# szumanski/Audio-Modem-Radio

Hardware: AMD Instinct MI355X
Metric: demod Msymbols/s (batch) + achieved HBM GB/s, QPSK@9600/96kHz, 1/2/4/8 GPU (higher is better)
Workload: dtype f64; 1 GPU; qpsk9600; global_batch=4096, batches_in_flight=16, steps_per_launch=1, streams_per_launch=4096, kernel_layout=lane, hw_queues=32

## Files before the change

audio-modem-radio_amd/build.py:

```python
from __future__ import annotations

import hashlib
import os
import subprocess
import sys

HERE = os.path.dirname(os.path.abspath(__file__))
CSRC = os.path.join(HERE, "csrc")
INCLUDE = os.path.join(os.path.dirname(HERE), "include")
LIB = os.path.join(HERE, "libamr.so")
LIB_ID = LIB + ".id"
SOURCES = ["psk_kernels.hip", "psk_lane_kernels.hip", "psk_split_kernels.hip", "psk_soft_kernels.hip", "psk8_kernels.hip", "util_kernels.hip", "fft_kernels.hip", "fsk_kernels.hip", "fsk_exact_kernels.hip", "pocketfft_kernels.hip", "frame_kernels.hip", "tx_kernels.hip",
           "hell_kernels.hip", "viterbi_kernels.hip", "rs_kernels.hip", "ofdm_kernels.hip", "ofdm_acq_kernels.hip", "dsss_kernels.hip", "dsss_acq_kernels.hip", "msk_kernels.hip", "msk_acq_kernels.hip", "tone8_kernels.hip", "tone8_acq_kernels.hip", "api.cpp", "tx_api.cpp", "hell_api.cpp",
           "viterbi_api.cpp", "rs_api.cpp", "ofdm_api.cpp", "dsss_api.cpp", "msk_api.cpp", "tone8_api.cpp", "fsk_api.cpp", "pocketfft_plan.cpp"]
HEADERS = ["amr_internal.h", "psk_common.h", "fft.h", "api_common.h", "plan_core.h", "sym_plan.h", "tx_host.h", "env_switch.h", "dev_mem.h", "fsk_exact.h", "pocketfft.h", "pocketfft_dev.h",
           "iir_design.h", "split_chain.h", "split_bound.h", "odd_ext.h", "split_strict.h", "hell.h", "hell_glyphs.h", "viterbi.h", "rs.h", "ofdm.h", "dsss.h", "msk.h", "tone8.h", os.path.join(INCLUDE, "amr.h")]
ARCH = os.environ.get("AMR_OFFLOAD_ARCH", "gfx950")
HIPCC = os.environ.get("HIPCC", "/opt/rocm/bin/hipcc")
CFLAGS = ["-O3", "-std=c++17", "-fPIC", "-ffp-contract=off", "-fno-fast-math", f"--offload-arch={ARCH}",
          "-I", CSRC, "-I", INCLUDE, "-Wall", "-Wno-unused-function"]


def _digest(paths, extra: str = "") -> str:
    h = hashlib.sha256()
    for p in paths:
        with open(p, "rb") as f:
            h.update(os.path.basename(p).encode() + b"\0" + f.read())
    h.update(extra.encode())
    return h.hexdigest()[:16]

# ... 65 lines not shown
```

audio-modem-radio_amd/csrc/api.cpp:

```cpp
#include <hip/hip_runtime.h>
#include <rccl/rccl.h>

#include <algorithm>
#include <cmath>
#include <cstdio>
#include <cstdlib>
#include <cstring>
#include <mutex>
#include <optional>
#include <string>
#include <tuple>
#include <vector>

#include "amr_internal.h"
#include "api_common.h"
#include "dev_mem.h"
#include "iir_design.h"
#include "plan_core.h"
#include "split_strict.h"

namespace amr {
hipError_t launch_psk_bandpass(const PskBuffers&, const PskParams&, const Iir&, hipStream_t);
hipError_t launch_psk_lowpass_fwd(const PskBuffers&, const PskParams&, const Iir&, hipStream_t);
hipError_t launch_psk_lowpass_bwd(const PskBuffers&, const PskParams&, const Iir&, hipStream_t);
hipError_t launch_psk_lowpass_exact(const PskBuffers&, const PskParams&, const Iir&, hipStream_t);
hipError_t launch_psk_slice(const PskBuffers&, const PskParams&, hipStream_t, bool only_flagged = false);
hipError_t launch_psk_soft(const PskBuffers&, const PskParams&, int8_t*, int64_t, hipStream_t);
hipError_t launch_psk_slice8(const PskBuffers&, const PskParams&, hipStream_t, bool only_flagged = false);
hipError_t launch_psk_soft8(const PskBuffers&, const PskParams&, int8_t*, int64_t, hipStream_t);
hipError_t launch_psk_bandpass_lane(const PskBuffers&, const PskParams&, const Iir&, hipStream_t);
hipError_t launch_psk_bandpass_fixup(const PskBuffers&, const PskParams&, const Iir&, hipStream_t);
bool psk_lane_fused(const PskBuffers&, const PskParams&);
hipError_t launch_psk_lowpass_lane(const PskBuffers&, const PskParams&, const Iir&, hipStream_t, bool* sliced, int* kernel);
int64_t psk_lane_bp_scratch_doubles(int64_t n_streams, int64_t n, int pad);
int64_t psk_lane_lp_scratch_doubles(int64_t n_streams, int64_t n, int pad);
int64_t psk_exact_scratch_bytes(int64_t n_streams, int64_t m2);
hipError_t launch_synth_tile_noise(const float*, int64_t, int64_t, float*, int64_t, int64_t, float, uint64_t,
                                   hipStream_t);
hipError_t launch_sync_pack_gated(const uint32_t*, int64_t, int64_t, int64_t, uint8_t*, int64_t, int64_t*, int64_t*,
                                  const int32_t*, hipStream_t);
hipError_t launch_psk_split_bp(const PskBuffers&, const PskParams&, const Iir&, const PskSplit&, hipStream_t);
hipError_t launch_psk_split_lp(const PskBuffers&, const PskParams&, const Iir&, const PskSplit&, hipStream_t);
hipError_t launch_psk_split_slice(const PskBuffers&, const PskParams&, const PskSplit&, hipStream_t);
hipError_t launch_fec_decode(const uint8_t*, int64_t, const int64_t*, int64_t, uint8_t*, int64_t, int64_t*,
                             int32_t*, const uint32_t*, const uint32_t*, hipStream_t);
hipError_t launch_frame_parse(const uint8_t*, int64_t, const int64_t*, int64_t, int64_t, int32_t*, amr_frame_rec*,
                              const uint32_t*, const uint32_t*, hipStream_t);
}
// ... 943 lines not shown
    HIP_TRY(psk_slice_kind(b, pl->p, st));
    if (!gated) HIP_TRY(gate_wait(pl->gate, st));
    HIP_TRY(psk_sync_pack(pl, c.io, b.words, b.gate));
    if (c.soft.ptr) HIP_TRY(psk_soft_kind(b, pl->p, c.soft.ptr, c.soft.stride, st));
    return AMR_OK;
  });
}

int run_psk_lane(amr_psk_plan* pl, const PskCall& c, PskBuffers b) {
  hipStream_t st = pl->stream;
  static const bool f32f_env = env_on("AMR_PSK_F32F");
  static const bool nofix = env_on("AMR_PSK_F32F_NOFIX");
  b.fpeak = reinterpret_cast<double*>(pl->mem.split_peak.as<unsigned long long>());
  b.f32f = f32f_env && pl->p.f32_margin > 0.0 && !pl->lp_exact_only && psk_lane_fused(b, pl->p) ? 1 : 0;
  pl->last_f32f = b.f32f != 0;
  HIP_TRY_TIMED(*pl, AMR_T_BANDPASS, launch_psk_bandpass_lane(b, pl->p, pl->bp, st));
  bool sliced = false;
  if (pl->lp_exact_only) {
    HIP_TRY(hipMemsetD32Async((hipDeviceptr_t)b.flags, 1, (size_t)c.io.B, st));
  } else {
    HIP_TRY_TIMED(*pl, AMR_T_LOWPASS_FWD, launch_psk_lowpass_lane(b, pl->p, pl->lp, st, &sliced, &pl->last_lowpass));
  }
  if (int rc = timed(*pl, AMR_T_LOWPASS_EXACT, [&]() -> int {
        if (b.f32f && !nofix) HIP_TRY(launch_psk_bandpass_fixup(b, pl->p, pl->bp, st));
        HIP_TRY(launch_psk_lowpass_exact(b, pl->p, pl->lp, st));
        return AMR_OK;
      }))
    return rc;
  return timed(*pl, AMR_T_SYNC_PACK, [&]() -> int {
    HIP_TRY(psk_slice_kind(b, pl->p, st, sliced));
// ... 565 lines not shown
```

audio-modem-radio_amd/csrc/psk_kernels.hip:

```cpp
#include <math.h>
#include <stdlib.h>

#include <type_traits>

#include "amr_internal.h"
#include "psk_common.h"

namespace amr {

constexpr int kTileBytes = 256;
constexpr int kTilePitch = kTileBytes + 16;
constexpr int kBwdChunk = 32;

template <int CTRL>
__device__ __forceinline__ double dpp_f64(double v) {
  const long long u = __builtin_bit_cast(long long, v);
  const int lo = __builtin_amdgcn_mov_dpp((int)(u & 0xffffffff), CTRL, 0xF, 0xF, true);
  const int hi = __builtin_amdgcn_mov_dpp((int)(u >> 32), CTRL, 0xF, 0xF, true);
  return __builtin_bit_cast(double, ((long long)hi << 32) | (unsigned)lo);
}
constexpr int kQuadBcast0 = 0x00;

constexpr int kRowStreams = 4;
constexpr int kBpRing = 8;
// ... 729 lines not shown
        load(rr_[u]);
        __builtin_amdgcn_sched_barrier(0);
      }
    }
#pragma unroll
    for (int u = 0; u < R; ++u)
      if (cc - u >= 0) run(rr_[u], cc - u);
  }
  for (int jj = pad - 1; jj >= 0; --jj) {
    const double y = quad5_step(c, z, s3[s3q_index(w, comp, m2_pairs, jj + qs, sq)]);
    acc = tiny_min3(acc, y, y);
  }
  quad_flag(buf, s, j, !(acc >= kTinyHi) || !__builtin_isfinite(z));
}

template <int NT>
__device__ __forceinline__ void df2t_cplx_step(double (&zr)[NT - 1], double (&zc)[NT - 1],
                                               const double (&b)[NT], const double (&a)[NT],
                                               double x0, double x1, double& y0, double& y1) {
  const double t0x = 0.0 * x1, t1x = 0.0 * x0;
  y0 = zr[0] + (b[0] * x0 - t0x);
  y1 = zc[0] + (t1x + b[0] * x1);
  const double t0y = 0.0 * y1, t1y = 0.0 * y0;
#pragma unroll
  for (int i = 0; i < NT - 2; ++i) {
    const double r = zr[i + 1] + (b[i + 1] * x0 - t0x);
    const double m = zc[i + 1] + (t1x + b[i + 1] * x1);
    zr[i] = r - (a[i + 1] * y0 - t0y);
    zc[i] = m - (t1y + a[i + 1] * y1);
  }
  zr[NT - 2] = (b[NT - 1] * x0 - t0x) - (a[NT - 1] * y0 - t0y);
  zc[NT - 2] = (t1x + b[NT - 1] * x1) - (t1y + a[NT - 1] * y1);
}

__device__ __forceinline__ void cmul_np(double ar, double ai, double br, double bi, double& re, double& im) {
  re = __builtin_fma(ar, br, -(ai * bi));
  im = __builtin_fma(ar, bi, ai * br);
}

constexpr int kExactSlots = 128;
constexpr int kExactTile = 32;
int64_t psk_exact_slots(int64_t n_streams) {
  const int64_t g = (n_streams + kWave - 1) / kWave;
  return g < kExactSlots ? g : kExactSlots;
}
int64_t psk_exact_scratch_bytes(int64_t n_streams, int64_t m2) {
  const int64_t tiles = (m2 + kExactTile - 1) / kExactTile;
  return psk_exact_slots(n_streams) * tiles * 8 * kWave * 8;
}

template <int NT>
__global__ __launch_bounds__(64) void k_lowpass_exact(PskBuffers buf, PskParams p, Iir f) {
  if (buf.gate && *buf.gate == 0) return;
  static_assert(NT == 5, "checkpoint layout holds 2 x 4 states");
  const int lane = threadIdx.x;
  const int64_t n_groups = (buf.n_streams + kWave - 1) / kWave;
  const int64_t n = p.n;
  const int64_t n2 = (n + 1) >> 1;
  const int pad = p.pad2;
  const int64_t m2 = p.m2;
  const int64_t S = p.n_sym;
  const int64_t tiles = (m2 + kExactTile - 1) / kExactTile;
  const double4* __restrict__ lo = reinterpret_cast<const double4*>(buf.lo);
  double* __restrict__ ck = buf.s3 + (size_t)blockIdx.x * tiles * 8 * kWave + lane;
  double* __restrict__ sym = buf.s1;
  __shared__ double2 tile_out[kExactTile][kWave];
  for (int64_t g = blockIdx.x; g < n_groups; g += gridDim.x) {
    const int64_t s = g * kWave + lane;
    const bool live = s < buf.n_streams && buf.flags[s] != 0;
    if (!__any(live)) continue;

    double b[NT], a[NT], zr[NT - 1], zc[NT - 1];
#pragma unroll
    for (int i = 0; i < NT; ++i) { b[i] = f.b[i]; a[i] = f.a[i]; }

    auto bb = [&](int64_t i) -> double2 {
      const double fv = buf.s2[f_index(g, n2, i, lane)];
      const double4 l = lo[i];
      return make_double2(__builtin_fma(fv, l.x, l.y), __builtin_fma(fv, l.z, l.w));
    };
    const double2 x0 = bb(0), xl = bb(n - 1);
    double l2r, l2i, r2r, r2i;
    cmul_np(2.0, 0.0, x0.x, x0.y, l2r, l2i);
    cmul_np(2.0, 0.0, xl.x, xl.y, r2r, r2i);
    auto ext = [&](int64_t j) -> double2 {
      if (j < pad) { const double2 v = bb(pad - j); return make_double2(l2r - v.x, l2i - v.y); }
      if (j < pad + n) return bb(j - pad);
      const double2 v = bb(n - 2 - (j - pad - n));
      return make_double2(r2r - v.x, r2i - v.y);
    };
    {
      const double2 e0 = ext(0);
#pragma unroll
      for (int i = 0; i < NT - 1; ++i) cmul_np(f.zi[i], 0.0, e0.x, e0.y, zr[i], zc[i]);
    }
    double y0 = 0, y1 = 0;
    for (int64_t t = 0; t < tiles; ++t) {
      double* c = ck + (size_t)t * 8 * kWave;
#pragma unroll
      for (int i = 0; i < NT - 1; ++i) { c[i * kWave] = zr[i]; c[(NT - 1 + i) * kWave] = zc[i]; }
      const int64_t j1 = (t + 1) * kExactTile < m2 ? (t + 1) * kExactTile : m2;
      for (int64_t j = t * kExactTile; j < j1; ++j) {
        const double2 e = ext(j);
        df2t_cplx_step<NT>(zr, zc, b, a, e.x, e.y, y0, y1);
      }
    }
    double wr[NT - 1], wc[NT - 1];
#pragma unroll
    for (int i = 0; i < NT - 1; ++i) cmul_np(f.zi[i], 0.0, y0, y1, wr[i], wc[i]);

    int64_t k = S - 1;
    int64_t next_n = p.first + k * p.sps;
    for (int64_t t = tiles - 1; t >= 0; --t) {
      const double* c = ck + (size_t)t * 8 * kWave;
#pragma unroll
      for (int i = 0; i < NT - 1; ++i) { zr[i] = c[i * kWave]; zc[i] = c[(NT - 1 + i) * kWave]; }
      const int64_t j0 = t * kExactTile;
      const int64_t j1 = j0 + kExactTile < m2 ? j0 + kExactTile : m2;
      for (int64_t j = j0; j < j1; ++j) {
        const double2 e = ext(j);
        double o0, o1;
        df2t_cplx_step<NT>(zr, zc, b, a, e.x, e.y, o0, o1);
        tile_out[j - j0][lane] = make_double2(o0, o1);
      }
      for (int64_t j = j1 - 1; j >= j0; --j) {
        const double2 e = tile_out[j - j0][lane];
        double o0, o1;
        df2t_cplx_step<NT>(wr, wc, b, a, e.x, e.y, o0, o1);
        if (j - pad == next_n && k >= 0) {
          if (live) {
            sym[sym_index(s, S, k, 0)] = o0;
            sym[sym_index(s, S, k, 1)] = o1;
          }
          --k;
          next_n -= p.sps;
        }
      }
    }
  }
}

constexpr int kSliceWords = 32;
template <int WV>
__global__ __launch_bounds__(64 * WV) void k_slice(PskBuffers buf, PskParams p, int only_flagged) {
  if (buf.gate && *buf.gate == 0) return;
  constexpr int WPW = kSliceWords / WV;
  __shared__ uint32_t wl[kWave][kSliceWords + 1];
  const int lane = threadIdx.x & 63;
  const int wv = threadIdx.x >> 6;
  const int64_t s = (int64_t)blockIdx.y * kWave + lane;
  const bool live = s < buf.n_streams && (!only_flagged || buf.flags[s] != 0);
  const int64_t S = p.n_sym;
  const bool qpsk = p.kind == kQpsk;
// ... 120 lines not shown
```

audio-modem-radio_amd/csrc/psk_lane_kernels.hip:

```cpp
#include <math.h>

#include <type_traits>
#include <utility>

#include "amr.h"
#include "amr_internal.h"
#include "env_switch.h"
#include "psk_common.h"

namespace amr {

constexpr int kBpT = 32;
constexpr int kLpT = 40;
constexpr int kLpStaticFirstMax = 20;
constexpr int kLpCkReserveT = 20;


constexpr int kZoY = 1, kZoZ = 2;
template <int ZO>
__device__ __forceinline__ double bp_step(double (&z)[8], const Iir& f, double x, float& acc) {
  if constexpr (ZO == kZoZ) return df2t_step_zo(z, f, x, acc);
  else if constexpr (ZO == kZoY) return bp_step_zo(z, f, x);
  else return df2t_step<8>(z, f, x);
}
// ... 16 lines not shown
int64_t psk_lane_bp_scratch_doubles(int64_t n_streams, int64_t n, int pad) {
  const int64_t g = (n_streams + 63) / 64;
  return g * ((n / kBpT) * 8 + bp_lane_edge_cap(pad)) * 64;
}
int64_t psk_lane_lp_scratch_doubles(int64_t n_streams, int64_t n, int pad) {
  const int64_t g = (n_streams + 63) / 64;
  return 2 * g * ((n / kLpCkReserveT) * 4 + lp_lane_edge_cap(pad)) * 64;
}

template <typename T, int GPB, int ZO, bool FIXUP = false, bool F32F = false, int NT = 0>
__global__ __launch_bounds__(128 * GPB) void k_bp_lane2(PskBuffers buf, PskParams p, Iir f, int dev_fence) {
  static_assert(FIXUP ? GPB == 1 && !ZO && !F32F : GPB == 2,
                "two groups per workgroup, or the fix-up pass: one group, every tap, float64 f");
  static_assert(NT == 0 || !F32F, "cache policies: the float64 paths only");
  constexpr bool NTF = (NT & kNtFStore) != 0, NTC = (NT & kNtCk) != 0, NTX = (NT & kNtX) != 0;
  constexpr int TB = kBpT;
  constexpr int PER = 16 / (int)sizeof(T);
  constexpr int NL = TB / PER;
  static_assert(TB % PER == 0 && TB % 2 == 0, "tile = whole loads and whole pairs");
  __shared__ __attribute__((aligned(16))) double2 yb[GPB][2][TB / 2][64];
  const int lane = threadIdx.x & 63;
  const int wv = __builtin_amdgcn_readfirstlane(threadIdx.x >> 6);
  const int gi = wv >> 1, role = wv & 1;
  const int64_t w = (int64_t)blockIdx.x * GPB + gi;
  const bool active = w * 64 < buf.n_streams;
  const int64_t last = buf.n_streams - 1;
  const int64_t s = w * 64 + lane;
  if constexpr (FIXUP) {
    if (!active) return;
    if (!__syncthreads_or(s <= last && buf.bp_flags[s] != 0)) return;
// ... 52 lines not shown
        const double y1 = bp_step<ZO>(z, f, tile_x(cur, k + 1), acc);
        bp_watch<ZO>(acc, y0, y1);
      }
    }
    int e = 0;
    for (int64_t i = i_tail; i < n; ++i) {
      const double y = bp_step<ZO>(z, f, In<T>::cvt(x[i]), acc);
      bp_watch<ZO>(acc, y, y);
      st_pol<NTC>(&eb[(e++) * 64], y);
    }
    for (int jj = 0; jj < pad; ++jj) {
      const double y = bp_step<ZO>(z, f, ox.right(jj), acc);
      bp_watch<ZO>(acc, y, y);
      st_pol<NTC>(&eb[(e++) * 64], y);
    }
    if (bp_bad<ZO>(acc, z) && s <= last) atomicOr(&buf.bp_flags[s], 1);
    lane_pass_fence(dev_fence);
  }
  __syncthreads();

  if (role == 0) {
    v4u xr[NL];
    double cn[8];
    if (active && nt > 0) {
      load_tile(nt - 1, xr);
#pragma unroll
      for (int j = 0; j < 8; ++j) cn[j] = ld_pol<NTC>(&ck[((nt - 1) * 8 + j) * 64]);
    }
    for (int64_t it = 0; it <= nt; ++it) {
      const int64_t t = nt - 1 - it;
      if (active && t >= 0) {
// ... 16 lines not shown
          ybuf[k >> 1][lane] = make_double2(y0, y1);
        }
      }
      __syncthreads();
    }
  } else {
    double zb[8];
    float acc = __builtin_inff();
    unsigned long long pk = 0;
    auto pk_acc = [&](double y) {
      if constexpr (F32F) {
        const unsigned long long b = (unsigned long long)__double_as_longlong(y) & 0x7fffffffffffffffULL;
        pk = b > pk ? b : pk;
      }
    };
    if (active) {
      const double ylast = ld_pol<NTC>(&eb[(ne - 1) * 64]);
#pragma unroll
      for (int j = 0; j < 8; ++j) zb[j] = f.zi[j] * ylast;
      for (int e = ne - 1; e >= 0; --e) {
        const double y = bp_step<ZO>(zb, f, ld_pol<NTC>(&eb[e * 64]), acc);
        bp_watch<ZO>(acc, y, y);
        const int64_t i = i_tail + e;
        if (i < n) {
          if constexpr (F32F) {
            fo32[(i >> 1) * 64 + (i & 1)] = (float)y;
            pk_acc(y);
          } else {
            st_pol<NTF>(&fo[(i >> 1) * 64 + (i & 1)], y);
          }
        }
// ... 11 lines not shown
          const double2 yy = ybuf[k][lane];
          const double y1 = bp_step<ZO>(zb, f, yy.y, acc);
          const double y0 = bp_step<ZO>(zb, f, yy.x, acc);
          bp_watch<ZO>(acc, y1, y0);
          if constexpr (F32F) {
            *reinterpret_cast<float2*>(fp32 + k * 64) = make_float2((float)y0, (float)y1);
            pk_acc(y0);
            pk_acc(y1);
          } else {
            st_pair<NTF>(fp + k * 64, y0, y1);
          }
        }
      }
      __syncthreads();
    }
    if (active && bp_bad<ZO>(acc, zb) && s <= last) atomicOr(&buf.bp_flags[s], 1);
    if constexpr (F32F) {
      if (active && s <= last) buf.fpeak[s] = __longlong_as_double((long long)pk);
    }
  }
}

#ifndef AMR_LP_WAVES
#define AMR_LP_WAVES 1
#endif
#ifndef AMR_LP_CH
#define AMR_LP_CH 8
#endif
#ifndef AMR_LP_REGION_SYMS
#define AMR_LP_REGION_SYMS 8
#endif
template <int SPS, int FM, bool FUSE = false, bool F32F = false, int NT = 0>
__global__ __launch_bounds__(256, SPS > 0 ? AMR_LP_WAVES : 1) void k_lp_lane(PskBuffers buf, PskParams p, Iir f,
// ... 5 lines not shown
  static_assert(!F32F || FUSE, "the float32 hand-off's margin check runs in the fused slicer");
  using FV = typename std::conditional<F32F, float2, double2>::type;
  constexpr int TL = kLpT;
  constexpr int CH = AMR_LP_CH;
  constexpr int NCH = TL / CH, HC = CH / 2;
  constexpr int R = NCH % 2 == 0 ? NCH / 2 : NCH;
  static_assert(TL % CH == 0 && TL <= 64, "tile = whole chunks; one LO value per lane");
  static_assert(SPS == 0 || (TL % SPS == 0 && FM < SPS), "static symbol slots");
  __shared__ __attribute__((aligned(16))) double lo_lds[WPB][2][TL];
  constexpr int SPR = TL / (SPS > 0 ? SPS : TL);
  constexpr int MS = AMR_LP_REGION_SYMS;
  constexpr int RT = MS / SPR > 1 ? MS / SPR : 1;
  constexpr int NSL = FUSE ? 2 * MS : 1;
  static_assert(!FUSE || (RT * SPR <= MS && (MS & (MS - 1)) == 0), "a region holds at most MS symbols");
  __shared__ double sring[FUSE ? WPB : 1][NSL][64];
  const int lane = threadIdx.x & 63;
  const int wv = __builtin_amdgcn_readfirstlane(threadIdx.x >> 6);
  const int64_t w = (int64_t)blockIdx.x * (WPB / 2) + (wv >> 1);
  const int comp = wv & 1;
  const int64_t n = p.n, n2 = (n + 1) >> 1;
  const int pad = p.pad2;
  const int64_t nt = n / TL;
  if (w * 64 >= buf.n_streams) {
    if constexpr (FUSE) {
      for (int64_t b = 0; b < (nt > 1 ? (nt - 1 + RT - 1) / RT : 0) + 2; ++b) __syncthreads();
    }
    return;
  }
  const int64_t s = w * 64 + lane;
  const int64_t G = (buf.n_streams + 63) / 64;
// ... 223 lines not shown
        }
      }
      put_lo(tp, lop);
      if ((nt - 1 - t) % RT == RT - 1 || t == 1) {
        region_done(t * TL, r_hi);
        r_hi = t * TL;
      }
    }
  }
  for (int e = pad + (int)nh - 1; e >= 0; --e) {
    const double y = lp_step(zb, f, ld_pol<NTC>(&eh[e * 64]));
    accb = tiny_min3(accb, y, y);
    const int64_t i = e - pad;
    if (i >= 0) sym_out(i, y);
  }
  region_done(0, nh);
  bad |= !(accb >= kTinyHi);
#pragma unroll
  for (int j = 0; j < 4; ++j) bad |= !__builtin_isfinite(zb[j]);
  if constexpr (F32F) bad |= mflag;
  if (bad && s < buf.n_streams) {
    atomicOr(&buf.flags[s], 1);
    if constexpr (F32F) atomicOr(&buf.bp_flags[s], 1);
  }
}

template <int SPS, int FM, int NT = 0>
__global__ __launch_bounds__(256, AMR_LP_WAVES) void k_lp_lane_h(PskBuffers buf, PskParams p, Iir f, int dev_fence) {
  constexpr bool NTF = (NT & kNtFLoad) != 0, NTC = (NT & kNtCk) != 0, NTW = (NT & kNtWords) != 0;
  constexpr int TL = kLpT;
  constexpr int CH = AMR_LP_CH;
  constexpr int NCH = TL / CH, HC = CH / 2;
  constexpr int R = NCH % 2 == 0 ? NCH / 2 : NCH;
  static_assert(TL % CH == 0 && TL <= 64, "tile = whole chunks; one LO value of each component per lane");
  static_assert(SPS > 0 && TL % SPS == 0 && FM < SPS, "static symbol slots");
  __shared__ __attribute__((aligned(16))) double lo_lds[4][2][2][TL];
  const int lane = threadIdx.x & 63;
  const int hl = lane & 31, comp = lane >> 5;
// ... 205 lines not shown
        if (k % SPS == FM) slice(kt + (k - FM) / SPS, y1);
        if ((k - 1) % SPS == FM) slice(kt + (k - 1 - FM) / SPS, y0);
      }
      put_lo(tp, lop);
    }
  }
  for (int e = pad + (int)nh - 1; e >= 0; --e) {
    const double y = lp_step(zb, f, ld_pol<NTC>(&(eh + e * 64)[lane]));
    accb = tiny_min3(accb, y, y);
    const int64_t i = e - pad;
    if (i >= 0) sym_out(i, y);
  }
  bad |= !(accb >= kTinyHi);
#pragma unroll
  for (int j = 0; j < 4; ++j) bad |= !__builtin_isfinite(zb[j]);
  if (bad && live) atomicOr(&buf.flags[s], 1);
}


#ifndef AMR_LANE_NT_DEFAULT
#define AMR_LANE_NT_DEFAULT (kNtFStore | kNtFLoad | kNtCk)
#endif
#ifndef AMR_LANE_NT_MASKS
#define AMR_LANE_NT_MASKS 0, AMR_LANE_NT_DEFAULT, kNtAll
#endif
static int lane_nt() {
  static const int v = (int)env_int("AMR_LANE_NT", INT32_MIN, INT32_MAX, AMR_LANE_NT_DEFAULT);
  return v;
}
template <typename Fn, int... M>
static bool lane_nt_switch(int m, Fn&& fn, std::integer_sequence<int, M...>) {
  return ((m == M ? (fn(std::integral_constant<int, M>{}), true) : false) || ...);
}
// ... 8 lines not shown
}

static int bp_zero_taps(const PskParams& p) {
  static const bool on = env_not_off("AMR_BP_ZO");
  static const int det = env_not_off("AMR_BP_ZDET") ? kZoY : kZoZ;
  return on && p.bp_zero_odd && p.bp_sym ? det : 0;
}
template <typename Fn>
static void with_bp_zo(int zo, Fn&& fn) {
  if (zo == kZoY) fn(std::integral_constant<int, kZoY>{});
  else if (zo == kZoZ) fn(std::integral_constant<int, kZoZ>{});
  else fn(std::integral_constant<int, 0>{});
}

template <typename T>
static hipError_t launch_bp(const PskBuffers& b, const PskParams& p, const Iir& f, hipStream_t st) {
  const int64_t g = (b.n_streams + 63) / 64;
  const dim3 grid((unsigned)((g + 1) / 2)), block(256);
  if (b.f32f) {
    hipError_t e = hipMemsetAsync(b.bp_flags, 0, (size_t)b.n_streams * 4, st);
    if (e != hipSuccess) return e;
    with_bp_zo(bp_zero_taps(p), [&](auto z) {
      hipLaunchKernelGGL((k_bp_lane2<T, 2, decltype(z)::value, false, true>), grid, block, 0, st, b, p, f,
                         lane_dev_fence());
    });
    return hipGetLastError();
  }
  const int zo = bp_zero_taps(p);
  if (zo) {
    hipError_t e = hipMemsetAsync(b.bp_flags, 0, (size_t)b.n_streams * 4, st);
    if (e != hipSuccess) return e;
  }
  const bool ok = with_lane_nt([&](auto m) {
    constexpr int NT = decltype(m)::value;
    with_bp_zo(zo, [&](auto z) {
      hipLaunchKernelGGL((k_bp_lane2<T, 2, decltype(z)::value, false, false, NT>), grid, block, 0, st, b, p, f,
                         lane_dev_fence());
    });
    if (zo)
      hipLaunchKernelGGL((k_bp_lane2<T, 1, 0, true, false, NT>), dim3((unsigned)g), dim3(128), 0, st, b, p, f,
                         lane_dev_fence());
  });
  return ok ? hipGetLastError() : hipErrorInvalidValue;
}

hipError_t launch_psk_bandpass_lane(const PskBuffers& b, const PskParams& p, const Iir& f, hipStream_t st) {
  if (f.nt != 9) return hipErrorInvalidValue;
  switch (b.dtype) {
    case kF32: return launch_bp<float>(b, p, f, st);
    case kF64: return launch_bp<double>(b, p, f, st);
    case kI16: return launch_bp<int16_t>(b, p, f, st);
    default: return hipErrorInvalidValue;
  }
}

hipError_t launch_psk_bandpass_fixup(const PskBuffers& b, const PskParams& p, const Iir& f, hipStream_t st) {
  if (f.nt != 9) return hipErrorInvalidValue;
  const dim3 grid((unsigned)((b.n_streams + 63) / 64)), block(128);
  switch (b.dtype) {
    case kF32: hipLaunchKernelGGL((k_bp_lane2<float, 1, 0, true>), grid, block, 0, st, b, p, f, lane_dev_fence()); break;
    case kF64: hipLaunchKernelGGL((k_bp_lane2<double, 1, 0, true>), grid, block, 0, st, b, p, f, lane_dev_fence()); break;
    case kI16: hipLaunchKernelGGL((k_bp_lane2<int16_t, 1, 0, true>), grid, block, 0, st, b, p, f, lane_dev_fence()); break;
    default: return hipErrorInvalidValue;
  }
  return hipGetLastError();
}
// ... 45 lines not shown
  }
  const bool ok = with_lane_nt([&](auto m) {
    constexpr int NT = decltype(m)::value;
    if (fuse) hipLaunchKernelGGL((k_lp_lane<S_, F_, S_ != 0, false, NT>), grid, block, 0, st, b, p, f, lane_dev_fence());
    else hipLaunchKernelGGL((k_lp_lane<S_, F_, false, false, NT>), grid, block, 0, st, b, p, f, lane_dev_fence());
  });
  if (!ok) return -1;
  return fuse ? AMR_LP_LANE_FUSED : AMR_LP_LANE;
}

bool psk_lane_fused(const PskBuffers& b, const PskParams& p) {
  return with_lp_slots(p, [](auto s, auto) { return (int)decltype(s)::value; }) > 0 && lp_fuse_wanted(b);
}

hipError_t launch_psk_lowpass_lane(const PskBuffers& b, const PskParams& p, const Iir& f, hipStream_t st,
                                   bool* sliced, int* kernel) {
  if (f.nt != 5) return hipErrorInvalidValue;
  hipError_t e = hipMemsetAsync(b.flags, 0, (size_t)b.n_streams * 4, st);
  if (e != hipSuccess) return e;
  const int fused = with_lp_slots(p, [&](auto s, auto m) {
    return launch_lp<decltype(s)::value, decltype(m)::value>(b, p, f, st);
  });
  if (fused < 0) return hipErrorInvalidValue;
  if (sliced) *sliced = fused != AMR_LP_LANE;
  if (kernel) *kernel = fused;
  return hipGetLastError();
}

}
```

Measured before the change: 12040 Msym/s.

## Fuse band-pass fixup, exact lowpass and slicing into one lane epilogue kernel

Adds a deferred path for the fused lane pipeline. The band-pass and lowpass kernels now store their bad-stream flags directly instead of using atomicOr, which removes the two flag memsets. A single epilogue kernel then redoes the band-pass fixup and runs the exact lowpass with inline QPSK/BPSK slicing, but only for flagged stream groups. This replaces the separate fixup, exact-lowpass and slice launches and the symbol round-trip through memory. The trade-off is more complex kernels and reuse of shared-memory tiles. Correctness depends on the direct flag writes fully overwriting stale state.

```diff
diff --git a/audio-modem-radio_amd/build.py b/audio-modem-radio_amd/build.py
--- a/audio-modem-radio_amd/build.py
+++ b/audio-modem-radio_amd/build.py
@@ -13,7 +13,7 @@
 SOURCES = ["psk_kernels.hip", "psk_lane_kernels.hip", "psk_split_kernels.hip", "psk_soft_kernels.hip", "psk8_kernels.hip", "util_kernels.hip", "fft_kernels.hip", "fsk_kernels.hip", "fsk_exact_kernels.hip", "pocketfft_kernels.hip", "frame_kernels.hip", "tx_kernels.hip",
            "hell_kernels.hip", "viterbi_kernels.hip", "rs_kernels.hip", "ofdm_kernels.hip", "ofdm_acq_kernels.hip", "dsss_kernels.hip", "dsss_acq_kernels.hip", "msk_kernels.hip", "msk_acq_kernels.hip", "tone8_kernels.hip", "tone8_acq_kernels.hip", "api.cpp", "tx_api.cpp", "hell_api.cpp",
            "viterbi_api.cpp", "rs_api.cpp", "ofdm_api.cpp", "dsss_api.cpp", "msk_api.cpp", "tone8_api.cpp", "fsk_api.cpp", "pocketfft_plan.cpp"]
-HEADERS = ["amr_internal.h", "psk_common.h", "fft.h", "api_common.h", "plan_core.h", "sym_plan.h", "tx_host.h", "env_switch.h", "dev_mem.h", "fsk_exact.h", "pocketfft.h", "pocketfft_dev.h",
+HEADERS = ["amr_internal.h", "psk_common.h", "psk_exact.h", "fft.h", "api_common.h", "plan_core.h", "sym_plan.h", "tx_host.h", "env_switch.h", "dev_mem.h", "fsk_exact.h", "pocketfft.h", "pocketfft_dev.h",
            "iir_design.h", "split_chain.h", "split_bound.h", "odd_ext.h", "split_strict.h", "hell.h", "hell_glyphs.h", "viterbi.h", "rs.h", "ofdm.h", "dsss.h", "msk.h", "tone8.h", os.path.join(INCLUDE, "amr.h")]
 ARCH = os.environ.get("AMR_OFFLOAD_ARCH", "gfx950")
 HIPCC = os.environ.get("HIPCC", "/opt/rocm/bin/hipcc")
diff --git a/audio-modem-radio_amd/csrc/api.cpp b/audio-modem-radio_amd/csrc/api.cpp
--- a/audio-modem-radio_amd/csrc/api.cpp
+++ b/audio-modem-radio_amd/csrc/api.cpp
@@ -28,10 +28,13 @@
 hipError_t launch_psk_soft(const PskBuffers&, const PskParams&, int8_t*, int64_t, hipStream_t);
 hipError_t launch_psk_slice8(const PskBuffers&, const PskParams&, hipStream_t, bool only_flagged = false);
 hipError_t launch_psk_soft8(const PskBuffers&, const PskParams&, int8_t*, int64_t, hipStream_t);
-hipError_t launch_psk_bandpass_lane(const PskBuffers&, const PskParams&, const Iir&, hipStream_t);
+hipError_t launch_psk_bandpass_lane(const PskBuffers&, const PskParams&, const Iir&, hipStream_t, bool deferred = false);
 hipError_t launch_psk_bandpass_fixup(const PskBuffers&, const PskParams&, const Iir&, hipStream_t);
 bool psk_lane_fused(const PskBuffers&, const PskParams&);
-hipError_t launch_psk_lowpass_lane(const PskBuffers&, const PskParams&, const Iir&, hipStream_t, bool* sliced, int* kernel);
+hipError_t launch_psk_lowpass_lane(const PskBuffers&, const PskParams&, const Iir&, hipStream_t, bool* sliced, int* kernel,
+                                   bool deferred = false);
+bool psk_lane_epilogue_on();
+hipError_t launch_psk_lane_epilogue(const PskBuffers&, const PskParams&, const Iir& bp, const Iir& lp, hipStream_t);
 int64_t psk_lane_bp_scratch_doubles(int64_t n_streams, int64_t n, int pad);
 int64_t psk_lane_lp_scratch_doubles(int64_t n_streams, int64_t n, int pad);
 int64_t psk_exact_scratch_bytes(int64_t n_streams, int64_t m2);
@@ -1005,6 +1008,17 @@
   b.fpeak = reinterpret_cast<double*>(pl->mem.split_peak.as<unsigned long long>());
   b.f32f = f32f_env && pl->p.f32_margin > 0.0 && !pl->lp_exact_only && psk_lane_fused(b, pl->p) ? 1 : 0;
   pl->last_f32f = b.f32f != 0;
+  if (psk_lane_epilogue_on() && !b.f32f && !pl->lp_exact_only && psk_lane_fused(b, pl->p)) {
+    HIP_TRY_TIMED(*pl, AMR_T_BANDPASS, launch_psk_bandpass_lane(b, pl->p, pl->bp, st, true));
+    HIP_TRY_TIMED(*pl, AMR_T_LOWPASS_FWD,
+                  launch_psk_lowpass_lane(b, pl->p, pl->lp, st, nullptr, &pl->last_lowpass, true));
+    HIP_TRY_TIMED(*pl, AMR_T_LOWPASS_EXACT, launch_psk_lane_epilogue(b, pl->p, pl->bp, pl->lp, st));
+    return timed(*pl, AMR_T_SYNC_PACK, [&]() -> int {
+      HIP_TRY(gate_wait(pl->gate, st));
+      HIP_TRY(psk_sync_pack(pl, c.io, b.words));
+      return AMR_OK;
+    });
+  }
   HIP_TRY_TIMED(*pl, AMR_T_BANDPASS, launch_psk_bandpass_lane(b, pl->p, pl->bp, st));
   bool sliced = false;
   if (pl->lp_exact_only) {
diff --git a/audio-modem-radio_amd/csrc/psk_exact.h b/audio-modem-radio_amd/csrc/psk_exact.h
--- /dev/null
+++ b/audio-modem-radio_amd/csrc/psk_exact.h
@@ -0,0 +1,143 @@
+#pragma once
+#include "psk_common.h"
+
+namespace amr {
+
+template <int NT>
+__device__ __forceinline__ void df2t_cplx_step(double (&zr)[NT - 1], double (&zc)[NT - 1],
+                                               const double (&b)[NT], const double (&a)[NT],
+                                               double x0, double x1, double& y0, double& y1) {
+  const double t0x = 0.0 * x1, t1x = 0.0 * x0;
+  y0 = zr[0] + (b[0] * x0 - t0x);
+  y1 = zc[0] + (t1x + b[0] * x1);
+  const double t0y = 0.0 * y1, t1y = 0.0 * y0;
+#pragma unroll
+  for (int i = 0; i < NT - 2; ++i) {
+    const double r = zr[i + 1] + (b[i + 1] * x0 - t0x);
+    const double m = zc[i + 1] + (t1x + b[i + 1] * x1);
+    zr[i] = r - (a[i + 1] * y0 - t0y);
+    zc[i] = m - (t1y + a[i + 1] * y1);
+  }
+  zr[NT - 2] = (b[NT - 1] * x0 - t0x) - (a[NT - 1] * y0 - t0y);
+  zc[NT - 2] = (t1x + b[NT - 1] * x1) - (t1y + a[NT - 1] * y1);
+}
+
+__device__ __forceinline__ void cmul_np(double ar, double ai, double br, double bi, double& re, double& im) {
+  re = __builtin_fma(ar, br, -(ai * bi));
+  im = __builtin_fma(ar, bi, ai * br);
+}
+
+constexpr int kExactSlots = 128;
+constexpr int kExactTile = 32;
+
+template <int NT, bool SLICE>
+__device__ __forceinline__ void lowpass_exact_group(const PskBuffers& buf, const PskParams& p, const Iir& f, int64_t g,
+                                                    int lane, bool live, double* __restrict__ ck,
+                                                    double2 (*tile_out)[kWave]) {
+  static_assert(NT == 5, "checkpoint layout holds 2 x 4 states");
+  const int64_t s = g * kWave + lane;
+  const int64_t n = p.n;
+  const int64_t n2 = (n + 1) >> 1;
+  const int pad = p.pad2;
+  const int64_t m2 = p.m2;
+  const int64_t S = p.n_sym;
+  const int64_t tiles = (m2 + kExactTile - 1) / kExactTile;
+  const double4* __restrict__ lo = reinterpret_cast<const double4*>(buf.lo);
+  double* __restrict__ sym = buf.s1;
+
+  double b[NT], a[NT], zr[NT - 1], zc[NT - 1];
+#pragma unroll
+  for (int i = 0; i < NT; ++i) { b[i] = f.b[i]; a[i] = f.a[i]; }
+
+  auto bb = [&](int64_t i) -> double2 {
+    const double fv = buf.s2[f_index(g, n2, i, lane)];
+    const double4 l = lo[i];
+    return make_double2(__builtin_fma(fv, l.x, l.y), __builtin_fma(fv, l.z, l.w));
+  };
+  const double2 x0 = bb(0), xl = bb(n - 1);
+  double l2r, l2i, r2r, r2i;
+  cmul_np(2.0, 0.0, x0.x, x0.y, l2r, l2i);
+  cmul_np(2.0, 0.0, xl.x, xl.y, r2r, r2i);
+  auto ext = [&](int64_t j) -> double2 {
+    if (j < pad) { const double2 v = bb(pad - j); return make_double2(l2r - v.x, l2i - v.y); }
+    if (j < pad + n) return bb(j - pad);
+    const double2 v = bb(n - 2 - (j - pad - n));
+    return make_double2(r2r - v.x, r2i - v.y);
+  };
+  {
+    const double2 e0 = ext(0);
+#pragma unroll
+    for (int i = 0; i < NT - 1; ++i) cmul_np(f.zi[i], 0.0, e0.x, e0.y, zr[i], zc[i]);
+  }
+  double y0 = 0, y1 = 0;
+  for (int64_t t = 0; t < tiles; ++t) {
+    double* c = ck + (size_t)t * 8 * kWave;
+#pragma unroll
+    for (int i = 0; i < NT - 1; ++i) { c[i * kWave] = zr[i]; c[(NT - 1 + i) * kWave] = zc[i]; }
+    const int64_t j1 = (t + 1) * kExactTile < m2 ? (t + 1) * kExactTile : m2;
+    for (int64_t j = t * kExactTile; j < j1; ++j) {
+      const double2 e = ext(j);
+      df2t_cplx_step<NT>(zr, zc, b, a, e.x, e.y, y0, y1);
+    }
+  }
+  double wr[NT - 1], wc[NT - 1];
+#pragma unroll
+  for (int i = 0; i < NT - 1; ++i) cmul_np(f.zi[i], 0.0, y0, y1, wr[i], wc[i]);
+
+  int64_t k = S - 1;
+  int64_t next_n = p.first + k * p.sps;
+  [[maybe_unused]] double pr = 0.0, pim = 0.0;
+  [[maybe_unused]] uint32_t wacc = 0;
+  [[maybe_unused]] const bool qpsk = p.kind == kQpsk;
+  for (int64_t t = tiles - 1; t >= 0; --t) {
+    const double* c = ck + (size_t)t * 8 * kWave;
+#pragma unroll
+    for (int i = 0; i < NT - 1; ++i) { zr[i] = c[i * kWave]; zc[i] = c[(NT - 1 + i) * kWave]; }
+    const int64_t j0 = t * kExactTile;
+    const int64_t j1 = j0 + kExactTile < m2 ? j0 + kExactTile : m2;
+    for (int64_t j = j0; j < j1; ++j) {
+      const double2 e = ext(j);
+      double o0, o1;
+      df2t_cplx_step<NT>(zr, zc, b, a, e.x, e.y, o0, o1);
+      tile_out[j - j0][lane] = make_double2(o0, o1);
+    }
+    for (int64_t j = j1 - 1; j >= j0; --j) {
+      const double2 e = tile_out[j - j0][lane];
+      double o0, o1;
+      df2t_cplx_step<NT>(wr, wc, b, a, e.x, e.y, o0, o1);
+      if (j - pad == next_n && k >= 0) {
+        if constexpr (SLICE) {
+          if (k <= S - 2) {
+            const double br = o0, bi = -o1;
+            const double dr = __builtin_fma(pr, br, -(pim * bi));
+            if (qpsk) {
+              const double di = __builtin_fma(pr, bi, pim * br);
+              wacc |= qpsk_dibit(dr, di) << (30 - 2 * (int)(k & 15));
+              if ((k & 15) == 0) {
+                if (live) buf.words[(size_t)s * p.n_words + (k >> 4)] = wacc;
+                wacc = 0;
+              }
+            } else {
+              wacc |= (dr < 0 ? 1u : 0u) << (31 - (int)(k & 31));
+              if ((k & 31) == 0) {
+                if (live) buf.words[(size_t)s * p.n_words + (k >> 5)] = wacc;
+                wacc = 0;
+              }
+            }
+          }
+          pr = o0;
+          pim = o1;
+        } else {
+          if (live) {
+            sym[sym_index(s, S, k, 0)] = o0;
+            sym[sym_index(s, S, k, 1)] = o1;
+          }
+        }
+        --k;
+        next_n -= p.sps;
+      }
+    }
+  }
+}
+
+}
diff --git a/audio-modem-radio_amd/csrc/psk_kernels.hip b/audio-modem-radio_amd/csrc/psk_kernels.hip
--- a/audio-modem-radio_amd/csrc/psk_kernels.hip
+++ b/audio-modem-radio_amd/csrc/psk_kernels.hip
@@ -5,6 +5,7 @@
 
 #include "amr_internal.h"
 #include "psk_common.h"
+#include "psk_exact.h"
 
 namespace amr {
 
@@ -767,32 +768,6 @@
   quad_flag(buf, s, j, !(acc >= kTinyHi) || !__builtin_isfinite(z));
 }
 
-template <int NT>
-__device__ __forceinline__ void df2t_cplx_step(double (&zr)[NT - 1], double (&zc)[NT - 1],
-                                               const double (&b)[NT], const double (&a)[NT],
-                                               double x0, double x1, double& y0, double& y1) {
-  const double t0x = 0.0 * x1, t1x = 0.0 * x0;
-  y0 = zr[0] + (b[0] * x0 - t0x);
-  y1 = zc[0] + (t1x + b[0] * x1);
-  const double t0y = 0.0 * y1, t1y = 0.0 * y0;
-#pragma unroll
-  for (int i = 0; i < NT - 2; ++i) {
-    const double r = zr[i + 1] + (b[i + 1] * x0 - t0x);
-    const double m = zc[i + 1] + (t1x + b[i + 1] * x1);
-    zr[i] = r - (a[i + 1] * y0 - t0y);
-    zc[i] = m - (t1y + a[i + 1] * y1);
-  }
-  zr[NT - 2] = (b[NT - 1] * x0 - t0x) - (a[NT - 1] * y0 - t0y);
-  zc[NT - 2] = (t1x + b[NT - 1] * x1) - (t1y + a[NT - 1] * y1);
-}
-
-__device__ __forceinline__ void cmul_np(double ar, double ai, double br, double bi, double& re, double& im) {
-  re = __builtin_fma(ar, br, -(ai * bi));
-  im = __builtin_fma(ar, bi, ai * br);
-}
-
-constexpr int kExactSlots = 128;
-constexpr int kExactTile = 32;
 int64_t psk_exact_slots(int64_t n_streams) {
   const int64_t g = (n_streams + kWave - 1) / kWave;
   return g < kExactSlots ? g : kExactSlots;
@@ -805,91 +780,16 @@
 template <int NT>
 __global__ __launch_bounds__(64) void k_lowpass_exact(PskBuffers buf, PskParams p, Iir f) {
   if (buf.gate && *buf.gate == 0) return;
-  static_assert(NT == 5, "checkpoint layout holds 2 x 4 states");
   const int lane = threadIdx.x;
   const int64_t n_groups = (buf.n_streams + kWave - 1) / kWave;
-  const int64_t n = p.n;
-  const int64_t n2 = (n + 1) >> 1;
-  const int pad = p.pad2;
-  const int64_t m2 = p.m2;
-  const int64_t S = p.n_sym;
-  const int64_t tiles = (m2 + kExactTile - 1) / kExactTile;
-  const double4* __restrict__ lo = reinterpret_cast<const double4*>(buf.lo);
+  const int64_t tiles = (p.m2 + kExactTile - 1) / kExactTile;
   double* __restrict__ ck = buf.s3 + (size_t)blockIdx.x * tiles * 8 * kWave + lane;
-  double* __restrict__ sym = buf.s1;
   __shared__ double2 tile_out[kExactTile][kWave];
   for (int64_t g = blockIdx.x; g < n_groups; g += gridDim.x) {
     const int64_t s = g * kWave + lane;
     const bool live = s < buf.n_streams && buf.flags[s] != 0;
     if (!__any(live)) continue;
-
-    double b[NT], a[NT], zr[NT - 1], zc[NT - 1];
-#pragma unroll
-    for (int i = 0; i < NT; ++i) { b[i] = f.b[i]; a[i] = f.a[i]; }
-
-    auto bb = [&](int64_t i) -> double2 {
-      const double fv = buf.s2[f_index(g, n2, i, lane)];
-      const double4 l = lo[i];
-      return make_double2(__builtin_fma(fv, l.x, l.y), __builtin_fma(fv, l.z, l.w));
-    };
-    const double2 x0 = bb(0), xl = bb(n - 1);
-    double l2r, l2i, r2r, r2i;
-    cmul_np(2.0, 0.0, x0.x, x0.y, l2r, l2i);
-    cmul_np(2.0, 0.0, xl.x, xl.y, r2r, r2i);
-    auto ext = [&](int64_t j) -> double2 {
-      if (j < pad) { const double2 v = bb(pad - j); return make_double2(l2r - v.x, l2i - v.y); }
-      if (j < pad + n) return bb(j - pad);
-      const double2 v = bb(n - 2 - (j - pad - n));
-      return make_double2(r2r - v.x, r2i - v.y);
-    };
-    {
-      const double2 e0 = ext(0);
-#pragma unroll
-      for (int i = 0; i < NT - 1; ++i) cmul_np(f.zi[i], 0.0, e0.x, e0.y, zr[i], zc[i]);
-    }
-    double y0 = 0, y1 = 0;
-    for (int64_t t = 0; t < tiles; ++t) {
-      double* c = ck + (size_t)t * 8 * kWave;
-#pragma unroll
-      for (int i = 0; i < NT - 1; ++i) { c[i * kWave] = zr[i]; c[(NT - 1 + i) * kWave] = zc[i]; }
-      const int64_t j1 = (t + 1) * kExactTile < m2 ? (t + 1) * kExactTile : m2;
-      for (int64_t j = t * kExactTile; j < j1; ++j) {
-        const double2 e = ext(j);
-        df2t_cplx_step<NT>(zr, zc, b, a, e.x, e.y, y0, y1);
-      }
-    }
-    double wr[NT - 1], wc[NT - 1];
-#pragma unroll
-    for (int i = 0; i < NT - 1; ++i) cmul_np(f.zi[i], 0.0, y0, y1, wr[i], wc[i]);
-
-    int64_t k = S - 1;
-    int64_t next_n = p.first + k * p.sps;
-    for (int64_t t = tiles - 1; t >= 0; --t) {
-      const double* c = ck + (size_t)t * 8 * kWave;
-#pragma unroll
-      for (int i = 0; i < NT - 1; ++i) { zr[i] = c[i * kWave]; zc[i] = c[(NT - 1 + i) * kWave]; }
-      const int64_t j0 = t * kExactTile;
-      const int64_t j1 = j0 + kExactTile < m2 ? j0 + kExactTile : m2;
-      for (int64_t j = j0; j < j1; ++j) {
-        const double2 e = ext(j);
-        double o0, o1;
-        df2t_cplx_step<NT>(zr, zc, b, a, e.x, e.y, o0, o1);
-        tile_out[j - j0][lane] = make_double2(o0, o1);
-      }
-      for (int64_t j = j1 - 1; j >= j0; --j) {
-        const double2 e = tile_out[j - j0][lane];
-        double o0, o1;
-        df2t_cplx_step<NT>(wr, wc, b, a, e.x, e.y, o0, o1);
-        if (j - pad == next_n && k >= 0) {
-          if (live) {
-            sym[sym_index(s, S, k, 0)] = o0;
-            sym[sym_index(s, S, k, 1)] = o1;
-          }
-          --k;
-          next_n -= p.sps;
-        }
-      }
-    }
+    lowpass_exact_group<NT, false>(buf, p, f, g, lane, live, ck, tile_out);
   }
 }
 
diff --git a/audio-modem-radio_amd/csrc/psk_lane_kernels.hip b/audio-modem-radio_amd/csrc/psk_lane_kernels.hip
--- a/audio-modem-radio_amd/csrc/psk_lane_kernels.hip
+++ b/audio-modem-radio_amd/csrc/psk_lane_kernels.hip
@@ -7,6 +7,7 @@
 #include "amr_internal.h"
 #include "env_switch.h"
 #include "psk_common.h"
+#include "psk_exact.h"
 
 namespace amr {
 
@@ -54,6 +55,7 @@
                 "two groups per workgroup, or the fix-up pass: one group, every tap, float64 f");
   static_assert(NT == 0 || !F32F, "cache policies: the float64 paths only");
   constexpr bool NTF = (NT & kNtFStore) != 0, NTC = (NT & kNtCk) != 0, NTX = (NT & kNtX) != 0;
+  constexpr bool FST = ZO != 0 && !F32F;
   constexpr int TB = kBpT;
   constexpr int PER = 16 / (int)sizeof(T);
   constexpr int NL = TB / PER;
@@ -136,7 +138,8 @@
       bp_watch<ZO>(acc, y, y);
       st_pol<NTC>(&eb[(e++) * 64], y);
     }
-    if (bp_bad<ZO>(acc, z) && s <= last) atomicOr(&buf.bp_flags[s], 1);
+    if constexpr (FST) yb[gi][1][0][lane].x = bp_bad<ZO>(acc, z) ? 1.0 : 0.0;
+    else if (bp_bad<ZO>(acc, z) && s <= last) atomicOr(&buf.bp_flags[s], 1);
     lane_pass_fence(dev_fence);
   }
   __syncthreads();
@@ -183,7 +186,9 @@
         pk = b > pk ? b : pk;
       }
     };
+    [[maybe_unused]] unsigned long long fwd_bad = 0;
     if (active) {
+      if constexpr (FST) fwd_bad = __ballot(yb[gi][1][0][lane].x != 0.0);
       const double ylast = ld_pol<NTC>(&eb[(ne - 1) * 64]);
 #pragma unroll
       for (int j = 0; j < 8; ++j) zb[j] = f.zi[j] * ylast;
@@ -225,9 +230,113 @@
       }
       __syncthreads();
     }
-    if (active && bp_bad<ZO>(acc, zb) && s <= last) atomicOr(&buf.bp_flags[s], 1);
+    if constexpr (FST) {
+      if (active && s <= last) buf.bp_flags[s] = bp_bad<ZO>(acc, zb) || ((fwd_bad >> lane) & 1) ? 1 : 0;
+    } else {
+      if (active && bp_bad<ZO>(acc, zb) && s <= last) atomicOr(&buf.bp_flags[s], 1);
+    }
     if constexpr (F32F) {
       if (active && s <= last) buf.fpeak[s] = __longlong_as_double((long long)pk);
+    }
+  }
+}
+
+template <typename T>
+__device__ __forceinline__ void bp_fixup_group(const PskBuffers& buf, const PskParams& p, const Iir& f, int dev_fence,
+                                               double2 (&yb)[2][kBpT / 2][64], int64_t w, int role, int lane) {
+  constexpr int TB = kBpT;
+  constexpr int PER = 16 / (int)sizeof(T);
+  constexpr int NL = TB / PER;
+  const int64_t last = buf.n_streams - 1;
+  const int64_t s = w * 64 + lane;
+  const T* __restrict__ x = reinterpret_cast<const T*>(buf.x) + (s < last ? s : last) * buf.x_stride;
+  const uint8_t* __restrict__ xb = reinterpret_cast<const uint8_t*>(x);
+  const int64_t n = p.n, n2 = (n + 1) >> 1;
+  const int pad = p.pad1;
+  const int64_t nt = n / TB;
+  const int64_t G = (buf.n_streams + 63) / 64;
+  const int64_t ecap = bp_lane_edge_cap(pad);
+  const int64_t i_tail = nt * TB;
+  const int ne = (int)(n - i_tail) + pad;
+  double* __restrict__ ck = buf.s1 + (size_t)w * nt * 8 * 64 + lane;
+  double* __restrict__ eb = buf.s1 + (size_t)G * nt * 8 * 64 + (size_t)w * ecap * 64 + lane;
+  double* __restrict__ fo = buf.s2 + (size_t)(w * 2 + (lane >> 5)) * n2 * 64 + (lane & 31) * 2;
+  auto load_tile = [&](int64_t t, v4u (&r)[NL]) {
+#pragma unroll
+    for (int k = 0; k < NL; ++k) r[k] = *reinterpret_cast<const v4u*>(xb + (size_t)t * TB * sizeof(T) + k * 16);
+  };
+  auto tile_x = [&](const v4u (&r)[NL], int k) -> double {
+    T v[PER];
+    __builtin_memcpy(v, &r[k / PER], 16);
+    return In<T>::cvt(v[k % PER]);
+  };
+
+  if (role == 0) {
+    double z[8];
+    const OddExt<T> ox(x, buf.edge, s < last ? s : last, n, pad);
+    {
+      const double e0 = ox.left(0);
+#pragma unroll
+      for (int j = 0; j < 8; ++j) z[j] = f.zi[j] * e0;
+    }
+    for (int jj = 0; jj < pad; ++jj) df2t_step<8>(z, f, ox.left(jj));
+    for (int64_t t = 0; t < nt; ++t) {
+#pragma unroll
+      for (int j = 0; j < 8; ++j) ck[(t * 8 + j) * 64] = z[j];
+      v4u cur[NL];
+      load_tile(t, cur);
+#pragma unroll
+      for (int k = 0; k < TB; ++k) df2t_step<8>(z, f, tile_x(cur, k));
+    }
+    int e = 0;
+    for (int64_t i = i_tail; i < n; ++i) eb[(e++) * 64] = df2t_step<8>(z, f, In<T>::cvt(x[i]));
+    for (int jj = 0; jj < pad; ++jj) eb[(e++) * 64] = df2t_step<8>(z, f, ox.right(jj));
+    lane_pass_fence(dev_fence);
+  }
+  __syncthreads();
+
+  if (role == 0) {
+    for (int64_t it = 0; it <= nt; ++it) {
+      const int64_t t = nt - 1 - it;
+      if (t >= 0) {
+        double zf[8];
+        v4u cur[NL];
+#pragma unroll
+        for (int j = 0; j < 8; ++j) zf[j] = ck[(t * 8 + j) * 64];
+        load_tile(t, cur);
+        double2 (*ybuf)[64] = yb[it & 1];
+#pragma unroll
+        for (int k = 0; k < TB; k += 2) {
+          const double y0 = df2t_step<8>(zf, f, tile_x(cur, k));
+          const double y1 = df2t_step<8>(zf, f, tile_x(cur, k + 1));
+          ybuf[k >> 1][lane] = make_double2(y0, y1);
+        }
+      }
+      __syncthreads();
+    }
+  } else {
+    double zb[8];
+    const double ylast = eb[(ne - 1) * 64];
+#pragma unroll
+    for (int j = 0; j < 8; ++j) zb[j] = f.zi[j] * ylast;
+    for (int e = ne - 1; e >= 0; --e) {
+      const double y = df2t_step<8>(zb, f, eb[e * 64]);
+      const int64_t i = i_tail + e;
+      if (i < n) fo[(i >> 1) * 64 + (i & 1)] = y;
+    }
+    __syncthreads();
+    for (int64_t it = 1; it <= nt; ++it) {
+      const int64_t t = nt - it;
+      const double2 (*ybuf)[64] = yb[(it - 1) & 1];
+      double* const fp = fo + (size_t)(t * (TB / 2)) * 64;
+#pragma unroll
+      for (int k = TB / 2 - 1; k >= 0; --k) {
+        const double2 yy = ybuf[k][lane];
+        const double y1 = df2t_step<8>(zb, f, yy.y);
+        const double y0 = df2t_step<8>(zb, f, yy.x);
+        st_pair<false>(fp + k * 64, y0, y1);
+      }
+      __syncthreads();
     }
   }
 }
@@ -263,6 +372,8 @@
   constexpr int NSL = FUSE ? 2 * MS : 1;
   static_assert(!FUSE || (RT * SPR <= MS && (MS & (MS - 1)) == 0), "a region holds at most MS symbols");
   __shared__ double sring[FUSE ? WPB : 1][NSL][64];
+  constexpr bool FST = FUSE && !F32F;
+  __shared__ int im_bad[FST ? WPB / 2 : 1][64];
   const int lane = threadIdx.x & 63;
   const int wv = __builtin_amdgcn_readfirstlane(threadIdx.x >> 6);
   const int64_t w = (int64_t)blockIdx.x * (WPB / 2) + (wv >> 1);
@@ -516,14 +627,21 @@
     const int64_t i = e - pad;
     if (i >= 0) sym_out(i, y);
   }
+  bad |= !(accb >= kTinyHi);
+#pragma unroll
+  for (int j = 0; j < 4; ++j) bad |= !__builtin_isfinite(zb[j]);
+  if constexpr (FST) {
+    if (comp == 1) im_bad[wv >> 1][lane] = bad ? 1 : 0;
+  }
   region_done(0, nh);
-  bad |= !(accb >= kTinyHi);
-#pragma unroll
-  for (int j = 0; j < 4; ++j) bad |= !__builtin_isfinite(zb[j]);
-  if constexpr (F32F) bad |= mflag;
-  if (bad && s < buf.n_streams) {
-    atomicOr(&buf.flags[s], 1);
-    if constexpr (F32F) atomicOr(&buf.bp_flags[s], 1);
+  if constexpr (FST) {
+    if (comp == 0 && s < buf.n_streams) buf.flags[s] = bad || im_bad[wv >> 1][lane] != 0 ? 1 : 0;
+  } else {
+    if constexpr (F32F) bad |= mflag;
+    if (bad && s < buf.n_streams) {
+      atomicOr(&buf.flags[s], 1);
+      if constexpr (F32F) atomicOr(&buf.bp_flags[s], 1);
+    }
   }
 }
 
@@ -759,9 +877,37 @@
   bad |= !(accb >= kTinyHi);
 #pragma unroll
   for (int j = 0; j < 4; ++j) bad |= !__builtin_isfinite(zb[j]);
-  if (bad && live) atomicOr(&buf.flags[s], 1);
-}
-
+  const unsigned long long bm = __ballot(bad);
+  if (wr) buf.flags[s] = (int32_t)(((unsigned)bm | (unsigned)(bm >> 32)) >> hl & 1u);
+}
+
+template <typename T>
+__global__ __launch_bounds__(128) void k_psk_lane_epilogue(PskBuffers buf, PskParams p, Iir fbp, Iir flp, int use_bp,
+                                                           int dev_fence) {
+  __shared__ __attribute__((aligned(16))) double2 yb[2][kBpT / 2][64];
+  static_assert(sizeof(yb) == sizeof(double2) * kExactTile * kWave, "K3x's tile aliases the band-pass tile buffers");
+  double2 (*tile_out)[kWave] = reinterpret_cast<double2 (*)[kWave]>(&yb[0][0][0]);
+  const int lane = threadIdx.x & 63;
+  const int wv = __builtin_amdgcn_readfirstlane(threadIdx.x >> 6);
+  const int64_t n_groups = (buf.n_streams + kWave - 1) / kWave;
+  const int64_t xtiles = (p.m2 + kExactTile - 1) / kExactTile;
+  double* __restrict__ xck = buf.s3 + (size_t)blockIdx.x * xtiles * 8 * kWave + lane;
+  for (int64_t g = blockIdx.x; g < n_groups; g += gridDim.x) {
+    const int64_t s = g * kWave + lane;
+    const bool in = s < buf.n_streams;
+    const bool bpf = use_bp && in && buf.bp_flags[s] != 0;
+    const bool redo = bpf || (in && buf.flags[s] != 0);
+    if (!__any(redo)) continue;
+    if (__any(bpf)) {
+      bp_fixup_group<T>(buf, p, fbp, dev_fence, yb, g, wv, lane);
+      __syncthreads();
+    }
+    if (wv == 0) lowpass_exact_group<5, true>(buf, p, flp, g, lane, redo, xck, tile_out);
+    __syncthreads();
+  }
+}
+
+int64_t psk_exact_slots(int64_t n_streams);
 
 #ifndef AMR_LANE_NT_DEFAULT
 #define AMR_LANE_NT_DEFAULT (kNtFStore | kNtFLoad | kNtCk)
@@ -800,7 +946,7 @@
 }
 
 template <typename T>
-static hipError_t launch_bp(const PskBuffers& b, const PskParams& p, const Iir& f, hipStream_t st) {
+static hipError_t launch_bp(const PskBuffers& b, const PskParams& p, const Iir& f, hipStream_t st, bool deferred) {
   const int64_t g = (b.n_streams + 63) / 64;
   const dim3 grid((unsigned)((g + 1) / 2)), block(256);
   if (b.f32f) {
@@ -813,7 +959,7 @@
     return hipGetLastError();
   }
   const int zo = bp_zero_taps(p);
-  if (zo) {
+  if (zo && !deferred) {
     hipError_t e = hipMemsetAsync(b.bp_flags, 0, (size_t)b.n_streams * 4, st);
     if (e != hipSuccess) return e;
   }
@@ -823,19 +969,20 @@
       hipLaunchKernelGGL((k_bp_lane2<T, 2, decltype(z)::value, false, false, NT>), grid, block, 0, st, b, p, f,
                          lane_dev_fence());
     });
-    if (zo)
+    if (zo && !deferred)
       hipLaunchKernelGGL((k_bp_lane2<T, 1, 0, true, false, NT>), dim3((unsigned)g), dim3(128), 0, st, b, p, f,
                          lane_dev_fence());
   });
   return ok ? hipGetLastError() : hipErrorInvalidValue;
 }
 
-hipError_t launch_psk_bandpass_lane(const PskBuffers& b, const PskParams& p, const Iir& f, hipStream_t st) {
-  if (f.nt != 9) return hipErrorInvalidValue;
+hipError_t launch_psk_bandpass_lane(const PskBuffers& b, const PskParams& p, const Iir& f, hipStream_t st,
+                                    bool deferred) {
+  if (f.nt != 9 || (deferred && b.f32f)) return hipErrorInvalidValue;
   switch (b.dtype) {
-    case kF32: return launch_bp<float>(b, p, f, st);
-    case kF64: return launch_bp<double>(b, p, f, st);
-    case kI16: return launch_bp<int16_t>(b, p, f, st);
+    case kF32: return launch_bp<float>(b, p, f, st, deferred);
+    case kF64: return launch_bp<double>(b, p, f, st, deferred);
+    case kI16: return launch_bp<int16_t>(b, p, f, st, deferred);
     default: return hipErrorInvalidValue;
   }
 }
@@ -911,10 +1058,14 @@
 }
 
 hipError_t launch_psk_lowpass_lane(const PskBuffers& b, const PskParams& p, const Iir& f, hipStream_t st,
-                                   bool* sliced, int* kernel) {
+                                   bool* sliced, int* kernel, bool deferred) {
   if (f.nt != 5) return hipErrorInvalidValue;
-  hipError_t e = hipMemsetAsync(b.flags, 0, (size_t)b.n_streams * 4, st);
-  if (e != hipSuccess) return e;
+  if (deferred) {
+    if (b.f32f || !psk_lane_fused(b, p)) return hipErrorInvalidValue;
+  } else {
+    hipError_t e = hipMemsetAsync(b.flags, 0, (size_t)b.n_streams * 4, st);
+    if (e != hipSuccess) return e;
+  }
   const int fused = with_lp_slots(p, [&](auto s, auto m) {
     return launch_lp<decltype(s)::value, decltype(m)::value>(b, p, f, st);
   });
@@ -924,4 +1075,23 @@
   return hipGetLastError();
 }
 
-}
+bool psk_lane_epilogue_on() {
+  static const bool v = env_not_off("AMR_LANE_EPILOGUE");
+  return v;
+}
+
+hipError_t launch_psk_lane_epilogue(const PskBuffers& b, const PskParams& p, const Iir& fbp, const Iir& flp,
+                                    hipStream_t st) {
+  if (fbp.nt != 9 || flp.nt != 5 || b.f32f) return hipErrorInvalidValue;
+  const dim3 grid((unsigned)psk_exact_slots(b.n_streams)), block(128);
+  const int use_bp = bp_zero_taps(p) != 0;
+  switch (b.dtype) {
+    case kF32: hipLaunchKernelGGL((k_psk_lane_epilogue<float>), grid, block, 0, st, b, p, fbp, flp, use_bp, lane_dev_fence()); break;
+    case kF64: hipLaunchKernelGGL((k_psk_lane_epilogue<double>), grid, block, 0, st, b, p, fbp, flp, use_bp, lane_dev_fence()); break;
+    case kI16: hipLaunchKernelGGL((k_psk_lane_epilogue<int16_t>), grid, block, 0, st, b, p, fbp, flp, use_bp, lane_dev_fence()); break;
+    default: return hipErrorInvalidValue;
+  }
+  return hipGetLastError();
+}
+
+}
```

Result: no change. 12100 Msym/s, median of 6 (+0.5%).
